# jyf588/SimGAN

Hardware: AMD Instinct MI355X
Metric: env-steps/sec of GAIL-dyn PPO update (higher is better)
Workload: dtype f32; 1 GPU; northstar: GAIL-dyn update, T=128 N=512/GPU obs=47 act=12 D-in=86 policy=mlp h64 D h100 ppo_epoch=10 num_mini_batch=1...; optimizer_steps_per_update=2720, parallelism=single GPU

## Files before the change

simgan_amd/csrc/sg_ppo.hip:

```cpp
#include <math.h>
#include <stdlib.h>
#include <string.h>

#include <algorithm>
#include <vector>

#include "sg_common.h"
#include "sg_rng.hpp"
#include "sg_ppo_kernels.hpp"
#include "sg_kfac.hpp"
#include "sg_gru_kernels.hpp"

__global__ void k_fill_perm(int64_t* perm, int64_t n, int half_bits, uint64_t key) {
    const int64_t i = (int64_t)blockIdx.x * blockDim.x + threadIdx.x;
    if (i < n) perm[i] = sg_perm_at(i, n, half_bits, key);
}

int sg_fill_perm(sg_ctx* ctx, int64_t* d_perm, int64_t n, uint64_t seed, uint64_t stream_id) {
    const uint64_t key = sg_key(seed, 0x5045524Dull, stream_id);
    hipLaunchKernelGGL(k_fill_perm, dim3((unsigned)((n + 255) / 256)), dim3(256), 0, ctx->stream, d_perm, n,
                       sg_perm_half_bits((uint64_t)n), key);
    SG_CHECK(hipGetLastError());
    return 0;
}

static int max_trunk_floats(const SgPolicyDesc& d) {
    int m = 0;
    for (int t = 0; t < d.n_trunks; ++t) m = d.trunk[t].size > m ? d.trunk[t].size : m;
    return m;
}
static int max_bwd_floats(const SgPolicyDesc& d) {
    int m = 0;
    for (int t = 0; t < d.n_trunks; ++t) { const int s = d.trunk[t].size - d.trunk[t].w2; m = s > m ? s : m; }
    return m;
}
static int stack_ldP(const SgPolicyDesc& d) {
    int m = 0;
    for (int t = 0; t < d.n_trunks; ++t) m = d.trunk[t].ldP > m ? d.trunk[t].ldP : m;
    return m;
}
static size_t ppo_fwd_lds(const SgPolicyDesc& d, int MT, bool gw) {
    const int R = 16 * MT;
    return sizeof(float) * ((gw ? 0 : (size_t)max_trunk_floats(d)) + R * d.ldO + 2 * R * d.ldH);
}
static bool ppo_fused(const SgPolicyDesc& d, int MT) {
    const char* e = getenv("SG_PPO_FUSED");
    return d.kind == SG_POLICY_MLP && MT <= 2 && !(e && !strcmp(e, "0"));
}
static size_t ppo_bwd_lds(const SgPolicyDesc& d, int MT, bool gw) {
    const int R = 16 * MT;
    return sizeof(float) * ((gw ? 0 : (size_t)(ppo_fused(d, MT) ? max_trunk_floats(d) : max_bwd_floats(d))) + R * d.ldO + 2 * R * d.ldH + 2 * R * stack_ldP(d) +
                            ((R * d.A + 3) & ~3) + 7 * R);
}
static size_t ppo_bwd_sym_lds(const SgPolicyDesc& d, int MT, bool gw) {
    const int R = 16 * MT;
    return sizeof(float) * ((gw ? 0 : (size_t)max_bwd_floats(d)) + R * d.ldO + 2 * R * d.ldH + 3 * R * stack_ldP(d) +
                            ((R * d.A + 3) & ~3) + 7 * R + ((d.A * d.A + 3) & ~3));
}

static size_t a2c_bwd_lds(const SgPolicyDesc& d, int MT, bool gw) {
    const int R = 16 * MT;
    return sizeof(float) * ((gw ? 0 : (size_t)max_bwd_floats(d)) + R * d.ldO + 2 * R * d.ldH + 2 * R * stack_ldP(d) +
                            ((R * d.A + 3) & ~3) + 7 * R);
}
#define SG_A2C_CHUNK_ROWS 4096

#define SG_PPO_SHAPES(X) X(1, 3, 4) X(2, 3, 4)  X(2, 1, 7)  \
                         X(2, 4, 7)  X(2, 7, 4)

static int ppo_block_threads(int MT) {
    const char* we = getenv("SG_PPO_WAVES");
    return (MT >= 2 && !(we && atoi(we) == 4)) ? 512 : 256;
}

static void launch_ppo_fwd(sg_ctx* ctx, int MT, const SgPolicyDesc& d, dim3 grid, size_t lds, const PpoArgs& pa, bool gw) {
    const int ko = d.Op / 16, kh = d.Hc == d.H ? d.Hp / 16 : 0;
// ... 1059 lines not shown
            for (int k = 0; k < M; ++k) {
                step_off[(size_t)e * M + k] = (int)n_own;
                for (int64_t i = 0; i < mb_global; ++i) {
                    const int64_t g = perms[(size_t)e * TN_perm + (size_t)k * mb_global + i];
                    const int64_t t = g / Ng, c = g - t * Ng, owner = c / r->N;
                    if (owner == ctx->rank) {
                        SG_REQUIRE(n_own < TN, "sg_ppo_update: epoch %d hands this rank more than its %lld rows", e, (long long)TN);
                        own_perm[(size_t)e * TN + n_own++] = t * r->N + (c - owner * r->N);
                    }
                }
                const int cnt = (int)n_own - step_off[(size_t)e * M + k];
                step_cnt[(size_t)e * M + k] = cnt;
                if (cnt > mb) mb = cnt;
            }
            epoch_rows[e] = n_own;
        }
    } else {
        for (int e = 0; e < E; ++e)
            for (int k = 0; k < M; ++k) { step_cnt[(size_t)e * M + k] = mb; step_off[(size_t)e * M + k] = k * mb; }
    }

    const bool sym = a->sym_coef > 0.f;
    if (sym) {
        if (a->d_mobs_mat) {
            if (a->mrows_cap < TN * d.O) {
                SG_CHECK(hipStreamSynchronize(ctx->stream));
                if (a->d_mrows) SG_CHECK(sg_dev_free(a->d_mrows));
                SG_CHECK(sg_dev_malloc((void**)&a->d_mrows, sizeof(float) * TN * d.O));
                a->mrows_cap = TN * d.O;
            }
            hipLaunchKernelGGL(k_mirror_rows, dim3((unsigned)((TN * d.O + 255) / 256)), dim3(256), 0, ctx->stream,
                               r->d_field[SG_F_OBS], a->d_mobs_mat, a->d_mrows, TN, d.O);
            SG_CHECK(hipGetLastError());
        } else {
            SG_REQUIRE(a->mrows_host == TN * d.O, "sg_ppo_update: the symmetry loss takes its mirrored observations from the host: "
                       "sg_ppo_set_mirrored_obs must hand over %lld floats (T*N rows of %d) before every update (pending: %lld)",
                       (long long)(TN * d.O), d.O, (long long)a->mrows_host);
            a->mrows_host = 0;
        }
    }

    float* adv = r->d_field[SG_F_ADVANTAGES];
    double* stats = a->d_loss_acc + 4;
    hipLaunchKernelGGL(k_adv_stats, dim3(1), dim3(1024), 0, ctx->stream, r->d_field[SG_F_RETURNS],
                       r->d_field[SG_F_VALUE_PREDS], TN, adv, stats, 0);
    if (ctx->use_comm) SG_TRY(sg_comm_allreduce_f64(ctx, stats, 3));
    hipLaunchKernelGGL(k_adv_stats, dim3(1), dim3(1024), 0, ctx->stream, r->d_field[SG_F_RETURNS],
                       r->d_field[SG_F_VALUE_PREDS], TN, adv, stats, 1);
    if (ctx->use_comm) SG_TRY(sg_comm_allreduce_f64(ctx, stats + 1, 1));
    hipLaunchKernelGGL(k_adv_stats, dim3(64), dim3(1024), 0, ctx->stream, r->d_field[SG_F_RETURNS],
                       r->d_field[SG_F_VALUE_PREDS], TN, adv, stats, 2);
    SG_CHECK(hipGetLastError());

    if (a->perms_cap < (int64_t)E * TN) {
        SG_CHECK(hipStreamSynchronize(ctx->stream));
        if (a->d_perms) SG_CHECK(sg_dev_free(a->d_perms));
        SG_CHECK(sg_dev_malloc((void**)&a->d_perms, sizeof(int64_t) * (size_t)E * TN));
        a->perms_cap = (int64_t)E * TN;
    }
    a->last_perm_count = owned ? 0 : (int64_t)E * TN;
    if (owned) {
        SG_CHECK(hipMemcpyAsync(a->d_perms, own_perm.data(), sizeof(int64_t) * (size_t)E * TN, hipMemcpyHostToDevice, ctx->stream));
        SG_CHECK(hipStreamSynchronize(ctx->stream));
    } else if (perms) {
        SG_CHECK(hipMemcpyAsync(a->d_perms, perms, sizeof(int64_t) * (size_t)E * TN, hipMemcpyHostToDevice, ctx->stream));
        if (!out3) SG_CHECK(hipStreamSynchronize(ctx->stream));
    } else {
        for (int e = 0; e < E; ++e)
            SG_TRY(sg_fill_perm(ctx, a->d_perms + (size_t)e * TN, TN, seed, (uint64_t)e * 2654435761ull + (uint64_t)ctx->rank));
    }

    const int ncols = d.n_trunks + (sym ? 1 : 0);
    int MT = ((size_t)((mb + 15) / 16) * (size_t)(d.total + 8) * sizeof(float) > ((size_t)24 << 20) ||
              ((mb + 31) / 32) * ncols >= ctx->num_cu) ? 2 : 1;
    if (const char* e = getenv("SG_PPO_ROWS")) {
        const int v = atoi(e);
        if (v == 16 || v == 32 || v == 64) MT = v / 16;
    }
    const bool gw = sg_policy_needs_gw(ctx, d) || ppo_fwd_lds(d, 1, false) > (size_t)ctx->lds_bytes ||
                    ppo_bwd_lds(d, 1, false) > (size_t)ctx->lds_bytes || (sym && ppo_bwd_sym_lds(d, 1, false) > (size_t)ctx->lds_bytes);
    if ((gw || sym) && MT > 2) MT = 2;
    while (MT > 1 && (ppo_fwd_lds(d, MT, gw) > (size_t)ctx->lds_bytes || ppo_bwd_lds(d, MT, gw) > (size_t)ctx->lds_bytes ||
                      (sym && ppo_bwd_sym_lds(d, MT, gw) > (size_t)ctx->lds_bytes))) MT /= 2;
    const int R = 16 * MT;
    const int G = (mb + R - 1) / R;
    const int mbp = G * R;
    const int ldP = stack_ldP(d);
    const int slab_stride = (d.total + 8 + 63) & ~63;
    const int TNp = (int)TN + 64 + (owned ? mbp : 0);

    const size_t slab_f = (size_t)(sym ? 2 : 1) * G * slab_stride;
    const size_t xm_off = ((size_t)TNp * (d.ldO + d.A + 4) + 3) & ~(size_t)3;
    const size_t epoch_f = sym ? xm_off + (size_t)TNp * d.ldO : (size_t)TNp * (d.ldO + d.A + 4);
    const size_t stack_f = (size_t)ncols * mbp * (2 * (size_t)d.ldH + ldP);
    if (a->slabs_cap < slab_f || a->stacks_cap < epoch_f + stack_f) {
        SG_CHECK(hipStreamSynchronize(ctx->stream));
        if (a->d_slabs) SG_CHECK(sg_dev_free(a->d_slabs));
        if (a->d_stacks) SG_CHECK(sg_dev_free(a->d_stacks));
        SG_CHECK(sg_dev_malloc((void**)&a->d_slabs, sizeof(float) * slab_f));
        SG_CHECK(sg_dev_malloc((void**)&a->d_stacks, sizeof(float) * (epoch_f + stack_f)));
        a->slabs_cap = slab_f;
        a->stacks_cap = epoch_f + stack_f;
        a->scratch_key = 0;
    }
    const uint64_t key = ((uint64_t)G << 40) ^ ((uint64_t)slab_stride << 20) ^ ((uint64_t)mbp << 8) ^ (uint64_t)TNp ^ ((uint64_t)MT << 60) ^
                         ((uint64_t)sym << 63);
    if (a->scratch_key != key) {
        SG_CHECK(hipMemsetAsync(a->d_slabs, 0, sizeof(float) * slab_f, ctx->stream));
        SG_CHECK(hipMemsetAsync(a->d_stacks, 0, sizeof(float) * (epoch_f + stack_f), ctx->stream));
        a->scratch_key = key;
    }
    hipLaunchKernelGGL(k_zero_f64, dim3(1), dim3(64), 0, ctx->stream, a->d_loss_acc, 4);

    float* epX = a->d_stacks;
    float* epACT = epX + (size_t)TNp * d.ldO;
    float* epSC = epACT + (size_t)TNp * d.A;
    float* epXm = sym ? a->d_stacks + xm_off : nullptr;
    float* stk = a->d_stacks + epoch_f;

    EpochGatherArgs ga;
    ga.obs = r->d_field[SG_F_OBS]; ga.actions = r->d_field[SG_F_ACTIONS]; ga.old_logp = r->d_field[SG_F_LOGP];
    ga.adv = adv; ga.vpred = r->d_field[SG_F_VALUE_PREDS]; ga.ret = r->d_field[SG_F_RETURNS];
    ga.TN = TN; ga.O = d.O; ga.Op = d.Op; ga.ldO = d.ldO; ga.A = d.A; ga.sc_stride = TNp;
    ga.X = epX; ga.ACT = epACT; ga.SC = epSC;
    ga.mobs = sym ? a->d_mrows : nullptr; ga.Xm = epXm;

    PpoArgs pa;
    pa.d = d; pa.params = a->policy->d_params;
    pa.sc_stride = TNp; pa.mb = mb; pa.mbp = mbp; pa.inv_B = 1.0f / (float)mb_global;
    pa.clip = a->cfg.clip_param; pa.vcoef = a->cfg.value_loss_coef; pa.ecoef = a->cfg.entropy_coef;
    pa.use_clipped = a->cfg.use_clipped_value_loss;
    pa.slabs = a->d_slabs; pa.slab_stride = slab_stride; pa.ldP = ldP; pa.dbg = a->d_dbg;
    pa.st = reinterpret_cast<SgOptState*>(a->d_state); pa.G = G; pa.k1 = 0;
    pa.pair = a->d_pair;
    pa.Xm = nullptr; pa.MA = a->d_mact;
    pa.sym_c = sym ? (float)(2.0 * a->sym_coef / ((double)mb_global * d.A)) : 0.f;
    for (int t = 0; t < 3; ++t) {
        const bool on = t < ncols;
        pa.H1[t] = on ? stk : nullptr; if (on) stk += (size_t)mbp * d.ldH;
        pa.H2[t] = on ? stk : nullptr; if (on) stk += (size_t)mbp * d.ldH;
        pa.OUT[t] = on ? stk : nullptr; if (on) stk += (size_t)mbp * ldP;
    }
    const int wb_f = gw ? 0 : max_trunk_floats(d), wb_b = gw ? 0 : max_bwd_floats(d);
    const bool fused = !sym && ppo_fused(d, MT);
    const size_t lds_fc = sizeof(float) * ((size_t)wb_f + R * d.ldO + 2 * R * d.ldH + 2 * R * ldP + ((R * d.A + 3) & ~3) + 7 * R);
    const char* cfenv = getenv("SG_PPO_CRITIC_FIRST");
    const bool crit_first = !gw && !fused && d.kind == SG_POLICY_SPLIT && MT <= 2 && lds_fc <= (size_t)ctx->lds_bytes &&
                            (cfenv ? cfenv[0] == '1' : G * d.n_trunks > ctx->num_cu);
    const char* penv = getenv("SG_PPO_PAIR");
    const bool pair = !gw && !fused && !crit_first && d.kind == SG_POLICY_SPLIT && d.n_trunks == 3 && MT <= 2 &&
                      lds_fc <= (size_t)ctx->lds_bytes && 3 * G <= ctx->num_cu && 2 * ldP + 2 <= std::min(d.trunk[0].ldH, d.trunk[1].ldH) && !a->d_dbg &&
                      !a->self_wait_failed && (penv ? strcmp(penv, "0") != 0 : sg_ctx_exclusive(ctx));
    if (pair && !a->pair_primed) SG_CHECK(hipMemsetAsync(a->d_stacks, 0, sizeof(float) * (epoch_f + stack_f), ctx->stream));
    a->pair_primed = pair;
    const size_t lds_f = ppo_fwd_lds(d, MT, gw), lds_b = sym ? ppo_bwd_sym_lds(d, MT, gw) : ppo_bwd_lds(d, MT, gw);
    const int nblk = (d.total + 8 + 255) / 256;
    const int nblk_r = (d.total + 8 + SG_PPO_REDUCE_PARAMS - 1) / SG_PPO_REDUCE_PARAMS;
    SgOptState* st = reinterpret_cast<SgOptState*>(a->d_state);

    auto enqueue_steps = [&]() -> int {
        hipLaunchKernelGGL(k_opt_prepare_first, dim3(1), dim3(1), 0, ctx->stream, st);
        for (int e = 0; e < E; ++e) {
            ga.perm = a->d_perms + (size_t)e * TN;
            ga.TN = epoch_rows[e];
            if (ga.TN) hipLaunchKernelGGL(sym ? k_ppo_epoch_gather_sym : k_ppo_epoch_gather, dim3((unsigned)((ga.TN + 63) / 64)), dim3(256), 0,
                                          ctx->stream, ga);
            for (int k = 0; k < M; ++k) {
                const size_t rb = (size_t)step_off[(size_t)e * M + k];
                pa.mb = step_cnt[(size_t)e * M + k];
                pa.X = epX + rb * d.ldO; pa.ACT = epACT + rb * d.A; pa.SC = epSC + rb;
                if (sym) pa.Xm = epXm + rb * d.ldO;
                pa.k1 = e * M + k + 1;
                if (sym) {
                    pa.wbuf_floats = wb_f;
                    launch_ppo_fwd_sym(ctx, MT, d, dim3(G, 3), lds_f, pa, gw);
                    pa.wbuf_floats = wb_b;
                    launch_ppo_bwd_sym(ctx, MT, d, dim3(G, 3), lds_b, pa, gw);
                } else if (pair) {
                    pa.wbuf_floats = wb_f;
                    launch_ppo_pair(ctx, MT, d, G, lds_fc, pa);
                } else if (crit_first) {
                    pa.wbuf_floats = wb_f;
                    launch_ppo_fwd_critic(ctx, MT, d, dim3(G, d.n_trunks), lds_fc > lds_f ? lds_fc : lds_f, pa);
                    pa.wbuf_floats = wb_b;
                    launch_ppo_bwd(ctx, MT, d, dim3(G, d.n_trunks - 1), lds_b, pa, false, false);
                } else {
                    if (!fused) {
                        pa.wbuf_floats = wb_f;
                        launch_ppo_fwd(ctx, MT, d, dim3(G, d.n_trunks), lds_f, pa, gw);
                    }
                    pa.wbuf_floats = fused ? wb_f : wb_b;
                    launch_ppo_bwd(ctx, MT, d, dim3(G, d.n_trunks), lds_b, pa, fused, gw);
                }
                if (sym) SG_LAUNCH(ctx, SG_PROF_PPO_REDUCE, k_ppo_reduce_sym, dim3(nblk_r), dim3(256), 0, a->d_slabs, G, slab_stride,
                                   d.total, a->d_grad, a->d_part, d.trunk[0].off, d.trunk[0].off + d.trunk[0].ex);
                else SG_LAUNCH(ctx, SG_PROF_PPO_REDUCE, k_ppo_reduce, dim3(nblk_r), dim3(256), 0, a->d_slabs, G, slab_stride,
                               d.total, a->d_grad, a->d_part);
                if (ctx->use_comm) {
                    SG_TRY(sg_comm_allreduce_f32(ctx, a->d_grad, d.total + 8));
                    hipLaunchKernelGGL(k_sumsq, dim3(nblk), dim3(256), 0, ctx->stream, a->d_grad, d.total, a->d_part);
                }
                SG_LAUNCH(ctx, SG_PROF_PPO_ADAM, sym ? k_ppo_adam_sym : k_ppo_adam, dim3(nblk), dim3(256), 0, a->policy->d_params, a->d_m,
                          a->d_v, a->d_grad, a->d_part, ctx->use_comm ? nblk : nblk_r, d.total, st, e * M + k + 1, a->cfg.eps,
                          a->cfg.max_grad_norm, pa.inv_B, a->d_loss_acc);
            }
        }
        hipLaunchKernelGGL(k_opt_commit, dim3(1), dim3(1), 0, ctx->stream, st, E * M);
        return 0;
    };
    const char* genv = getenv("SG_PPO_GRAPH");
    const char* gcenv = getenv("SG_PPO_GRAPH_COMM");
    const bool comm_ok = !a->graph_refused && (!ctx->use_comm || (sg_comm_graph_ok(ctx) && !(gcenv && !strcmp(gcenv, "0"))));
    bool use_graph = comm_ok && !owned && !ctx->profile && !a->d_dbg && !(genv && !strcmp(genv, "0"));
    if (use_graph) {
        uint32_t fbits[6];
        const float fv[6] = {a->cfg.clip_param, a->cfg.value_loss_coef, a->cfg.entropy_coef, a->cfg.eps, a->cfg.max_grad_norm, pa.inv_B};
        memcpy(fbits, fv, sizeof fbits);
        uint32_t cbits;
        memcpy(&cbits, &a->sym_coef, sizeof cbits);
        const uint64_t key[18] = {(uint64_t)(uintptr_t)a->d_slabs, (uint64_t)(uintptr_t)a->d_stacks, (uint64_t)(uintptr_t)a->d_perms,
                                  (uint64_t)(uintptr_t)r->d_field[SG_F_OBS], (uint64_t)(uintptr_t)r->d_field[SG_F_ACTIONS],
                                  (uint64_t)(uintptr_t)r->d_field[SG_F_RETURNS], (uint64_t)(uintptr_t)a->policy->d_params,
                                  (uint64_t)TN, ((uint64_t)E << 32) | (uint64_t)M, ((uint64_t)MT << 32) | (uint64_t)G,
                                  ((uint64_t)fbits[0] << 32) | fbits[1], ((uint64_t)fbits[2] << 32) | fbits[3],
                                  ((uint64_t)fbits[4] << 32) | fbits[5], (uint64_t)a->cfg.use_clipped_value_loss,
                                  (uint64_t)(uintptr_t)r->d_field[SG_F_LOGP], 0x50504full + (fused ? 1 : 0) + (ctx->use_comm ? 2 : 0) + (crit_first ? 4 : 0) + (gw ? 8 : 0) + (pair ? 16 : 0) + (sg_comm_peer_on(ctx) ? 32 : 0) + (sym ? 64 : 0) + ((uint64_t)sg_comm_peer_generation(ctx) << 32),
                                  sym ? (uint64_t)(uintptr_t)a->d_mrows : 0, sym ? (uint64_t)cbits : 0};
        if (!a->steps_graph || memcmp(key, a->steps_graph_key, sizeof key) != 0) {
            if (a->steps_graph) { SG_CHECK(hipGraphExecDestroy(a->steps_graph)); a->steps_graph = nullptr; }
            if (sg_try_capture(ctx, &a->steps_graph, enqueue_steps) != 0) {
                a->graph_refused = true;
                use_graph = false;
            } else {
                memcpy(a->steps_graph_key, key, sizeof key);
            }
        }
        if (use_graph) SG_CHECK(hipGraphLaunch(a->steps_graph, ctx->stream));
    }
    if (!use_graph) SG_TRY(enqueue_steps());
    SG_CHECK(hipGetLastError());
    a->opt_t += (int64_t)E * M;
    if (!out3) return 0;
    double acc[3];
    SG_TRY(sg_ctx_fetch_f64(ctx, a->d_loss_acc, acc, 3));
    if (pair && (acc[0] != acc[0] || acc[1] != acc[1] || acc[2] != acc[2])) {
        unsigned err = 0;
        SG_COPY_SYNC(ctx, &err, a->d_pair + SG_PAIR_ERR_WORD, sizeof err, hipMemcpyDeviceToHost);
        if (err) {
            SG_CHECK(hipMemsetAsync(a->d_pair + SG_PAIR_ERR_WORD, 0, sizeof err, ctx->stream));
            a->self_wait_failed = true;
            SG_REQUIRE(false, "sg_ppo_update: a workgroup of k_ppo_pair waited %d s for its partner's words and gave "
                       "up (the policy's state is undefined; SG_PPO_PAIR=0 runs the multi-launch step)", (int)(SG_PAIR_TIMEOUT_TICKS / 100000000ll));
        }
    }
    const double nu = (double)E * M;
    for (int i = 0; i < 3; ++i) out3[i] = (float)(acc[i] / nu);
    return 0;
}

__global__ void k_publish(double* dst, const double* d_acc, const double* d_scal, const double* p_acc, double n_d, double n_p,
                          const unsigned* d_err, const unsigned* a_err, const unsigned* peer_err) {
    const int t = threadIdx.x;
    if (t < 3) dst[t] = d_acc ? d_acc[t] : 0.0;
    else if (t < 8) dst[t] = d_scal ? d_scal[t - 3] : 0.0;
    else if (t < 11) dst[t] = p_acc ? p_acc[t - 8] : 0.0;
    else if (t == 11) dst[t] = n_d;
    else if (t == 12) dst[t] = n_p;
    else if (t == 13) dst[t] = d_err ? (double)*d_err : 0.0;
    else if (t == 14) dst[t] = a_err ? (double)*a_err : 0.0;
    else if (t == 15) dst[t] = peer_err ? (double)__hip_atomic_load(peer_err, __ATOMIC_RELAXED, __HIP_MEMORY_SCOPE_AGENT) : 0.0;
}

extern "C" int sg_results_publish(sg_ctx* ctx, sg_disc* d, sg_ppo* a, int slot) {
    SG_REQUIRE(ctx && slot >= 0 && slot < SG_RESULT_SLOTS, "sg_results_publish: bad argument");
    SG_REQUIRE((!d || d->ctx == ctx) && (!a || a->ctx == ctx), "sg_results_publish: objects of another context");
    SG_CHECK(hipSetDevice(ctx->device));
    hipLaunchKernelGGL(k_publish, dim3(1), dim3(64), 0, ctx->stream, ctx->results + 16 * slot, d ? d->d_loss_acc : nullptr,
                       d ? d->d_scal : nullptr, a ? a->d_loss_acc : nullptr, d ? (double)d->last_n_d : 1.0,
                       a ? (double)a->cfg.ppo_epoch * a->cfg.num_mini_batch : 1.0,
// ... 47 lines not shown
```

simgan_amd/csrc/sg_ppo_kernels.hpp:

```cpp
#pragma once
#include "sg_common.h"
#include "sg_thin.hpp"

#define HALF_LOG_2PI 0.91893853320467274178f

struct PpoArgs {
    SgPolicyDesc d;
    const float* params;
    const float* X;
    const float* ACT;
    const float* SC;
    int sc_stride;
    int mb, mbp;
    float inv_B;
    float clip, vcoef, ecoef;
    int use_clipped;
    float* H1[3];
    float* H2[3];
    float* OUT[3];
    float* slabs;
    int slab_stride;
    int ldP;
    int wbuf_floats;
    long long* dbg;
    SgOptState* st;
    int k1, G;
    unsigned* pair;
    const float* Xm;
    const float* MA;
    float sym_c;
    float* DX[2] = {nullptr, nullptr};
};

#define SG_PAIR_BYTES 64
#define SG_PAIR_TIMEOUT_TICKS 300000000ll



#define SG_LDS_SYNC() asm volatile("s_waitcnt lgkmcnt(0)\n\ts_barrier" ::: "memory")

#define SG_PPO_STAMP(n) do { if (a.dbg && threadIdx.x == 0 && blockIdx.y == 0) a.dbg[blockIdx.x * 16 + (n)] = clock64(); } while (0)
#define SG_PPO_WALL(n) do { if (a.dbg && threadIdx.x == 0 && blockIdx.y < 2) a.dbg[(blockIdx.x + 512 * blockIdx.y) * 16 + (n)] = wall_clock64(); } while (0)

struct EpochGatherArgs {
    const float *obs, *actions, *old_logp, *adv, *vpred, *ret;
    const int64_t* perm;
    int64_t TN;
    int O, Op, ldO, A, sc_stride;
    float *X, *ACT, *SC;
    const float* mobs;
    float* Xm;
};

template <bool SYM = false, bool ROLLOUT_ORDER = false>
__device__ __forceinline__ void sg_ppo_epoch_gather_body(const EpochGatherArgs& a) {
    __shared__ int IDX[64];
    const int tid = threadIdx.x;
    const int64_t row0 = (int64_t)blockIdx.x * 64;
    if (tid < 64) {
        const int64_t rr = row0 + tid;
        const int idx = rr < a.TN ? (ROLLOUT_ORDER ? (int)rr : (int)a.perm[rr]) : -1;
        IDX[tid] = idx;
        if (ROLLOUT_ORDER) {
            if (idx >= 0) a.SC[3 * (size_t)a.sc_stride + rr] = a.ret[idx];
        } else if (idx >= 0) {
            a.SC[0 * (size_t)a.sc_stride + rr] = a.old_logp[idx];
            a.SC[1 * (size_t)a.sc_stride + rr] = a.adv[idx];
            a.SC[2 * (size_t)a.sc_stride + rr] = a.vpred[idx];
            a.SC[3 * (size_t)a.sc_stride + rr] = a.ret[idx];
        }
    }
    __syncthreads();
    for (int base = tid; base < 64 * a.Op; base += 8 * blockDim.x) {
        float v[8];
#pragma unroll
        for (int u = 0; u < 8; ++u) {
            const int i = base + u * blockDim.x;
            const int r = i / a.Op, c = i - r * a.Op;
            v[u] = (i < 64 * a.Op && IDX[r] >= 0 && c < a.O) ? a.obs[(size_t)IDX[r] * a.O + c] : 0.f;
        }
#pragma unroll
        for (int u = 0; u < 8; ++u) {
            const int i = base + u * blockDim.x;
            if (i < 64 * a.Op && IDX[i / a.Op] >= 0) a.X[(size_t)(row0 + i / a.Op) * a.ldO + (i % a.Op)] = v[u];
        }
        if (SYM) {
#pragma unroll
            for (int u = 0; u < 8; ++u) {
                const int i = base + u * blockDim.x;
                const int r = i / a.Op, c = i - r * a.Op;
                v[u] = (i < 64 * a.Op && IDX[r] >= 0 && c < a.O) ? a.mobs[(size_t)IDX[r] * a.O + c] : 0.f;
            }
#pragma unroll
            for (int u = 0; u < 8; ++u) {
                const int i = base + u * blockDim.x;
                if (i < 64 * a.Op && IDX[i / a.Op] >= 0) a.Xm[(size_t)(row0 + i / a.Op) * a.ldO + (i % a.Op)] = v[u];
            }
        }
    }
    for (int i = tid; i < 64 * a.A; i += blockDim.x) {
        const int r = i / a.A, c = i - r * a.A;
        if (IDX[r] >= 0) a.ACT[(size_t)(row0 + r) * a.A + c] = a.actions[(size_t)IDX[r] * a.A + c];
    }
}

__global__ __launch_bounds__(256) void k_ppo_epoch_gather(EpochGatherArgs a) { sg_ppo_epoch_gather_body<false>(a); }
__global__ __launch_bounds__(256) void k_ppo_epoch_gather_sym(EpochGatherArgs a) { sg_ppo_epoch_gather_body<true>(a); }
__global__ __launch_bounds__(256) void k_a2c_gather(EpochGatherArgs a) { sg_ppo_epoch_gather_body<false, true>(a); }

__global__ __launch_bounds__(256) void k_mirror_rows(const float* obs, const float* m, float* out, int64_t rows, int O) {
    const int64_t idx = (int64_t)blockIdx.x * blockDim.x + threadIdx.x;
    if (idx >= rows * O) return;
    const int64_t r = idx / O;
    const int i = (int)(idx - r * O);
    const float* x = obs + r * O;
    const float* mi = m + (size_t)i * O;
    double s = 0.0;
    for (int j = 0; j < O; ++j) {
        const float w = mi[j];
        if (w != 0.f) s += (double)w * (double)x[j];
    }
    out[idx] = (float)s;
}

template <int MT, int KO, int KH, bool GW = false, bool SYM = false>
__device__ __forceinline__ void sg_ppo_fwd_body(const PpoArgs& a, const int t, const int bx) {
    extern __shared__ __attribute__((aligned(16))) float smem[];
    constexpr int R = 16 * MT;
    const SgPolicyDesc& d = a.d;
    const int tid = threadIdx.x;
    const bool mirror = SYM && t == 2;
    const SgTrunk tr = d.trunk[mirror ? 0 : t];
    const int Op = (KO > 0 && KH > 0) ? 16 * KO : d.Op, Hp = (KO > 0 && KH > 0) ? 16 * KH : tr.Hp;
    const int ldO = Op + 4, ldH = Hp + 4, ldP = a.ldP;
    const float* W = GW ? a.params + tr.off : smem;
    float* X = smem + a.wbuf_floats;
    float* H1 = X + R * ldO;
    float* H2 = H1 + R * ldH;
    const int row0 = bx * R;

    SG_PPO_STAMP(0);
    float4 wv[12];
    if (!GW) sg_stage_issue<12>(wv, a.params + tr.off, tr.size / 4);
    {
        const float4* gx = reinterpret_cast<const float4*>((mirror ? a.Xm : a.X) + (size_t)row0 * ldO);
        float4* lx = reinterpret_cast<float4*>(X);
        for (int i = tid; i < R * ldO / 4; i += blockDim.x) lx[i] = gx[i];
    }
    SG_PPO_STAMP(1);
    if (!GW) sg_stage_commit<12>(smem, wv, a.params + tr.off, tr.size / 4);
    __syncthreads();
    SG_PPO_STAMP(2);
    const float* b1 = W + tr.b1;
    const float* b2 = W + tr.b2;
    const float* bh = W + tr.bh;
    float* gH1 = a.H1[t] + (size_t)row0 * ldH;
    float* gH2 = a.H2[t] + (size_t)row0 * ldH;
    float* gOUT = a.OUT[t] + (size_t)row0 * ldP;
    sg_layer_nt_u<MT, GW>(X, ldO, W + tr.w1, ldO, Op, Hp, [&](int r, int c, float v) {
        const float h = sg_tanh(v + b1[c]);
        H1[r * ldH + c] = h;
// ... 407 lines not shown

template <int MT, int KO, int KH>
__global__ __launch_bounds__(512) void k_ppo_fwd_critic(PpoArgs a) {
    if (blockIdx.y == 0) sg_ppo_bwd_body<MT, KO, KH, true>(a, a.d.n_trunks - 1, blockIdx.x);
    else sg_ppo_fwd_body<MT, KO, KH>(a, blockIdx.y - 1, blockIdx.x);
}

#define SG_PPO_REDUCE_PARAMS 64
template <bool SYM, bool ACC = false>
__device__ __forceinline__ void sg_ppo_reduce_body(const float* slabs, int n_slabs_, int slab_stride, int total,
                                                   float* grad, float* part, int lo2, int hi2, int acc = 0) {
    __shared__ float red[4][64];
    const int lane = threadIdx.x & 63, wave = threadIdx.x >> 6;
    const int i = blockIdx.x * SG_PPO_REDUCE_PARAMS + lane;
    const int n_slabs = (SYM && i >= lo2 && i < hi2) ? 2 * n_slabs_ : n_slabs_;
    float g = 0.f;
    if (i < total + 8) {
        for (int s0 = wave; s0 < n_slabs; s0 += 64) {
            float t[16];
#pragma unroll
            for (int u = 0; u < 16; ++u) {
                const int sidx = s0 + 4 * u;
                t[u] = slabs[(size_t)(sidx < n_slabs ? sidx : s0) * slab_stride + i];
            }
#pragma unroll
            for (int u = 0; u < 16; ++u) g += (s0 + 4 * u < n_slabs) ? t[u] : 0.f;
        }
    }
    red[wave][lane] = g;
    __syncthreads();
    if (wave == 0) {
        g = (red[0][lane] + red[1][lane]) + (red[2][lane] + red[3][lane]);
        if (ACC && acc && i < total + 8) g += grad[i];
        if (i < total + 8) grad[i] = g;
        float sq = (i < total) ? g * g : 0.f;
        sq = sg_wave_sum(sq);
        if (lane == 0) part[blockIdx.x] = sq;
    }
}
__global__ __launch_bounds__(256) void k_ppo_reduce(const float* slabs, int n_slabs, int slab_stride, int total,
                                                    float* grad, float* part) {
    sg_ppo_reduce_body<false>(slabs, n_slabs, slab_stride, total, grad, part, 0, 0);
}
__global__ __launch_bounds__(256) void k_ppo_reduce_sym(const float* slabs, int n_slabs, int slab_stride, int total,
                                                        float* grad, float* part, int lo2, int hi2) {
    sg_ppo_reduce_body<true>(slabs, n_slabs, slab_stride, total, grad, part, lo2, hi2);
}
__global__ __launch_bounds__(256) void k_a2c_reduce(const float* slabs, int n_slabs, int slab_stride, int total,
                                                    float* grad, float* part, int acc) {
    sg_ppo_reduce_body<false, true>(slabs, n_slabs, slab_stride, total, grad, part, 0, 0, acc);
}

__global__ void k_opt_prepare_first(SgOptState* st) { sg_opt_prepare(st, st->t0 + 1); }

__global__ __launch_bounds__(256) void k_sumsq(const float* grad, int total, float* part) {
    const int i = blockIdx.x * blockDim.x + threadIdx.x;
    float sq = (i < total) ? grad[i] * grad[i] : 0.f;
    sq = sg_wave_sum(sq);
    __shared__ float ws[4];
    if ((threadIdx.x & 63) == 0) ws[threadIdx.x >> 6] = sq;
    __syncthreads();
    if (threadIdx.x == 0) part[blockIdx.x] = ws[0] + ws[1] + ws[2] + ws[3];
}

template <int NL>
__device__ __forceinline__ void sg_ppo_adam_body(float* params, float* m, float* v, const float* grad,
                                                 const float* part, int n_part, int total,
                                                 const SgOptState* st, int k1, float eps, float max_norm,
                                                 float inv_mb, double* loss_acc) {
    __shared__ float s_coef;
    const int t = st->t0 + k1;
    const float s_step_size = st->step_size2[t & 1], s_bc2_sqrt = st->bc2_sqrt2[t & 1];
    __shared__ float s_ws[4];
    {
        float s = 0.f;
        for (int j = threadIdx.x; j < n_part; j += 256) s += part[j];
        s = sg_wave_sum(s);
        if ((threadIdx.x & 63) == 0) s_ws[threadIdx.x >> 6] = s;
    }
    __syncthreads();
    if (threadIdx.x == 0) {
        const float norm = sqrtf((s_ws[0] + s_ws[1]) + (s_ws[2] + s_ws[3]));
        float coef = max_norm / (norm + 1e-6f);
        s_coef = coef > 1.f ? 1.f : coef;
    }
    __syncthreads();
    const int i = blockIdx.x * blockDim.x + threadIdx.x;
    if (i < total) {
        const float g = grad[i] * s_coef;
        float mi = m[i], vi = v[i];
        mi = mi + (g - mi) * (float)(1.0 - 0.9);
        vi = vi * (float)0.999 + (float)(1.0 - 0.999) * g * g;
        const float denom = sqrtf(vi) / s_bc2_sqrt + eps;
        params[i] = params[i] - s_step_size * (mi / denom);
        m[i] = mi;
        v[i] = vi;
    }
    if (blockIdx.x == 0 && threadIdx.x < NL)
        loss_acc[threadIdx.x] += (double)(grad[total + threadIdx.x] * inv_mb);
    if (blockIdx.x == 0 && threadIdx.x == 64) sg_opt_prepare(const_cast<SgOptState*>(st), t + 1);
}
__global__ __launch_bounds__(256) void k_ppo_adam(float* params, float* m, float* v, const float* grad,
                                                  const float* part, int n_part, int total,
                                                  const SgOptState* st, int k1, float eps, float max_norm,
                                                  float inv_mb, double* loss_acc) {
    sg_ppo_adam_body<3>(params, m, v, grad, part, n_part, total, st, k1, eps, max_norm, inv_mb, loss_acc);
}
__global__ __launch_bounds__(256) void k_ppo_adam_sym(float* params, float* m, float* v, const float* grad,
                                                      const float* part, int n_part, int total,
                                                      const SgOptState* st, int k1, float eps, float max_norm,
                                                      float inv_mb, double* loss_acc) {
    sg_ppo_adam_body<4>(params, m, v, grad, part, n_part, total, st, k1, eps, max_norm, inv_mb, loss_acc);
}

__global__ __launch_bounds__(256) void k_a2c_rmsprop(float* params, float* sq, const float* grad, const float* part, int n_part,
                                                     int total, const SgOptState* st, float alpha, float one_m_alpha, float eps,
                                                     float max_norm, float inv_b, double* loss_acc) {
    __shared__ float s_coef;
    __shared__ float s_ws[4];
    {
        float s = 0.f;
        for (int j = threadIdx.x; j < n_part; j += 256) s += part[j];
        s = sg_wave_sum(s);
        if ((threadIdx.x & 63) == 0) s_ws[threadIdx.x >> 6] = s;
    }
    __syncthreads();
    if (threadIdx.x == 0) {
        const float norm = sqrtf((s_ws[0] + s_ws[1]) + (s_ws[2] + s_ws[3]));
        const float coef = max_norm / (norm + 1e-6f);
        s_coef = coef > 1.f ? 1.f : coef;
    }
    __syncthreads();
    const int i = blockIdx.x * blockDim.x + threadIdx.x;
    if (i < total) {
        const float g = grad[i] * s_coef;
        const float s = sq[i] * alpha + one_m_alpha * g * g;
        params[i] = params[i] + (-st->lr) * (g / (sqrtf(s) + eps));
        sq[i] = s;
    }
    if (blockIdx.x == 0 && threadIdx.x < 3) loss_acc[threadIdx.x] += (double)(grad[total + threadIdx.x] * inv_b);
}

__global__ __launch_bounds__(1024) void k_adv_stats(const float* ret, const float* vpred, int64_t n, float* adv,
                                                    double* stats ,
                                                    int pass) {
    __shared__ double ws[16];
    __shared__ double s_mean;
    const int tid = threadIdx.x;
    if (pass == 0) {
        double s = 0.0;
        for (int64_t i = tid; i < n; i += blockDim.x) {
            const float a = ret[i] - vpred[i];
            adv[i] = a;
            s += (double)a;
        }
        s = sg_wave_sum(s);
        if ((tid & 63) == 0) ws[tid >> 6] = s;
        __syncthreads();
        if (tid == 0) {
            double t = 0.0;
// ... 29 lines not shown
```

Baseline: 2.519 million env-steps/s.

## Overlap next-epoch gather with Adam steps via double-buffered epoch scratch

Double-buffers the per-epoch gathered minibatch scratch and spreads the next epoch's gather blocks across the Adam kernel launches of the current epoch, so the separate gather launch at each epoch boundary disappears. It also fills all epoch permutations in one 2-D launch, merges loss-accumulator zeroing into the optimizer prologue kernel, and restructures the gather body so scalar and action loads are issued before the observation copy. The change costs extra scratch memory and adds blocks to the Adam launches, and it is gated by an environment variable that defaults on.

Result: no change. 2.524 million env-steps/s, median of 4 (+0.2%).

```diff
diff --git a/simgan_amd/csrc/sg_ppo.hip b/simgan_amd/csrc/sg_ppo.hip
--- a/simgan_amd/csrc/sg_ppo.hip
+++ b/simgan_amd/csrc/sg_ppo.hip
@@ -22,6 +22,26 @@
                        sg_perm_half_bits((uint64_t)n), key);
     SG_CHECK(hipGetLastError());
     return 0;
+}
+
+__global__ void k_fill_perms(int64_t* perm, int64_t n, int half_bits, uint64_t seed, uint64_t stream0, uint64_t stride) {
+    const int64_t i = (int64_t)blockIdx.x * blockDim.x + threadIdx.x;
+    const uint64_t key = sg_key(seed, 0x5045524Dull, stream0 + (uint64_t)blockIdx.y * stride);
+    if (i < n) perm[(int64_t)blockIdx.y * n + i] = sg_perm_at(i, n, half_bits, key);
+}
+
+static int sg_fill_perms(sg_ctx* ctx, int64_t* d_perm, int64_t n, int E, uint64_t seed, uint64_t stream0, uint64_t stride) {
+    hipLaunchKernelGGL(k_fill_perms, dim3((unsigned)((n + 255) / 256), (unsigned)E), dim3(256), 0, ctx->stream, d_perm, n,
+                       sg_perm_half_bits((uint64_t)n), seed, stream0, stride);
+    SG_CHECK(hipGetLastError());
+    return 0;
+}
+
+static int ppo_epoch_pipeline() {
+    const char* e = getenv("SG_PPO_EPOCH_PIPELINE");
+    if (!e) return 16;
+    const int v = atoi(e);
+    return v == 0 ? 0 : v == 64 ? 64 : 16;
 }
 
 static int max_trunk_floats(const SgPolicyDesc& d) {
@@ -1187,6 +1207,7 @@
                        r->d_field[SG_F_VALUE_PREDS], TN, adv, stats, 2);
     SG_CHECK(hipGetLastError());
 
+    const int pipe_rows = ppo_epoch_pipeline();
     if (a->perms_cap < (int64_t)E * TN) {
         SG_CHECK(hipStreamSynchronize(ctx->stream));
         if (a->d_perms) SG_CHECK(sg_dev_free(a->d_perms));
@@ -1200,6 +1221,8 @@
     } else if (perms) {
         SG_CHECK(hipMemcpyAsync(a->d_perms, perms, sizeof(int64_t) * (size_t)E * TN, hipMemcpyHostToDevice, ctx->stream));
         if (!out3) SG_CHECK(hipStreamSynchronize(ctx->stream));
+    } else if (pipe_rows) {
+        SG_TRY(sg_fill_perms(ctx, a->d_perms, TN, E, seed, (uint64_t)ctx->rank, 2654435761ull));
     } else {
         for (int e = 0; e < E; ++e)
             SG_TRY(sg_fill_perm(ctx, a->d_perms + (size_t)e * TN, TN, seed, (uint64_t)e * 2654435761ull + (uint64_t)ctx->rank));
@@ -1228,30 +1251,34 @@
     const size_t xm_off = ((size_t)TNp * (d.ldO + d.A + 4) + 3) & ~(size_t)3;
     const size_t epoch_f = sym ? xm_off + (size_t)TNp * d.ldO : (size_t)TNp * (d.ldO + d.A + 4);
     const size_t stack_f = (size_t)ncols * mbp * (2 * (size_t)d.ldH + ldP);
-    if (a->slabs_cap < slab_f || a->stacks_cap < epoch_f + stack_f) {
+    const bool pipe = pipe_rows && !sym && !owned && E > 1;
+    const size_t ep2_off = (epoch_f + stack_f + 63) & ~(size_t)63;
+    const size_t scratch_f = pipe ? ep2_off + epoch_f : epoch_f + stack_f;
+    if (a->slabs_cap < slab_f || a->stacks_cap < scratch_f) {
         SG_CHECK(hipStreamSynchronize(ctx->stream));
         if (a->d_slabs) SG_CHECK(sg_dev_free(a->d_slabs));
         if (a->d_stacks) SG_CHECK(sg_dev_free(a->d_stacks));
         SG_CHECK(sg_dev_malloc((void**)&a->d_slabs, sizeof(float) * slab_f));
-        SG_CHECK(sg_dev_malloc((void**)&a->d_stacks, sizeof(float) * (epoch_f + stack_f)));
+        SG_CHECK(sg_dev_malloc((void**)&a->d_stacks, sizeof(float) * scratch_f));
         a->slabs_cap = slab_f;
-        a->stacks_cap = epoch_f + stack_f;
+        a->stacks_cap = scratch_f;
         a->scratch_key = 0;
     }
     const uint64_t key = ((uint64_t)G << 40) ^ ((uint64_t)slab_stride << 20) ^ ((uint64_t)mbp << 8) ^ (uint64_t)TNp ^ ((uint64_t)MT << 60) ^
-                         ((uint64_t)sym << 63);
+                         ((uint64_t)sym << 63) ^ ((uint64_t)pipe << 59);
     if (a->scratch_key != key) {
         SG_CHECK(hipMemsetAsync(a->d_slabs, 0, sizeof(float) * slab_f, ctx->stream));
-        SG_CHECK(hipMemsetAsync(a->d_stacks, 0, sizeof(float) * (epoch_f + stack_f), ctx->stream));
+        SG_CHECK(hipMemsetAsync(a->d_stacks, 0, sizeof(float) * scratch_f, ctx->stream));
         a->scratch_key = key;
     }
-    hipLaunchKernelGGL(k_zero_f64, dim3(1), dim3(64), 0, ctx->stream, a->d_loss_acc, 4);
+    if (!pipe_rows) hipLaunchKernelGGL(k_zero_f64, dim3(1), dim3(64), 0, ctx->stream, a->d_loss_acc, 4);
 
     float* epX = a->d_stacks;
     float* epACT = epX + (size_t)TNp * d.ldO;
     float* epSC = epACT + (size_t)TNp * d.A;
     float* epXm = sym ? a->d_stacks + xm_off : nullptr;
     float* stk = a->d_stacks + epoch_f;
+    const size_t ep_flip = pipe ? ep2_off : 0;
 
     EpochGatherArgs ga;
     ga.obs = r->d_field[SG_F_OBS]; ga.actions = r->d_field[SG_F_ACTIONS]; ga.old_logp = r->d_field[SG_F_LOGP];
@@ -1294,16 +1321,29 @@
     SgOptState* st = reinterpret_cast<SgOptState*>(a->d_state);
 
     auto enqueue_steps = [&]() -> int {
-        hipLaunchKernelGGL(k_opt_prepare_first, dim3(1), dim3(1), 0, ctx->stream, st);
+        if (pipe_rows) hipLaunchKernelGGL(k_ppo_prologue, dim3(1), dim3(64), 0, ctx->stream, st, a->d_loss_acc, 4);
+        else hipLaunchKernelGGL(k_opt_prepare_first, dim3(1), dim3(1), 0, ctx->stream, st);
         for (int e = 0; e < E; ++e) {
+            const size_t cur = (e & 1) ? ep_flip : 0, nxt = ep_flip - cur;
             ga.perm = a->d_perms + (size_t)e * TN;
             ga.TN = epoch_rows[e];
-            if (ga.TN) hipLaunchKernelGGL(sym ? k_ppo_epoch_gather_sym : k_ppo_epoch_gather, dim3((unsigned)((ga.TN + 63) / 64)), dim3(256), 0,
-                                          ctx->stream, ga);
+            ga.X = epX + cur; ga.ACT = epACT + cur; ga.SC = epSC + cur;
+            if (ga.TN && (e == 0 || !pipe))
+                hipLaunchKernelGGL(sym ? k_ppo_epoch_gather_sym : k_ppo_epoch_gather, dim3((unsigned)((ga.TN + 63) / 64)), dim3(256), 0,
+                                   ctx->stream, ga);
+            EpochGatherArgs gn = ga;
+            int ride_blocks = 0, ride_per = 0;
+            if (pipe && e + 1 < E) {
+                gn.perm = a->d_perms + (size_t)(e + 1) * TN;
+                gn.TN = epoch_rows[e + 1];
+                gn.X = epX + nxt; gn.ACT = epACT + nxt; gn.SC = epSC + nxt;
+                ride_blocks = (int)((gn.TN + pipe_rows - 1) / pipe_rows);
+                ride_per = (ride_blocks + M - 1) / M;
+            }
             for (int k = 0; k < M; ++k) {
                 const size_t rb = (size_t)step_off[(size_t)e * M + k];
                 pa.mb = step_cnt[(size_t)e * M + k];
-                pa.X = epX + rb * d.ldO; pa.ACT = epACT + rb * d.A; pa.SC = epSC + rb;
+                pa.X = epX + cur + rb * d.ldO; pa.ACT = epACT + cur + rb * d.A; pa.SC = epSC + cur + rb;
                 if (sym) pa.Xm = epXm + rb * d.ldO;
                 pa.k1 = e * M + k + 1;
                 if (sym) {
@@ -1335,9 +1375,19 @@
                     SG_TRY(sg_comm_allreduce_f32(ctx, a->d_grad, d.total + 8));
                     hipLaunchKernelGGL(k_sumsq, dim3(nblk), dim3(256), 0, ctx->stream, a->d_grad, d.total, a->d_part);
                 }
-                SG_LAUNCH(ctx, SG_PROF_PPO_ADAM, sym ? k_ppo_adam_sym : k_ppo_adam, dim3(nblk), dim3(256), 0, a->policy->d_params, a->d_m,
-                          a->d_v, a->d_grad, a->d_part, ctx->use_comm ? nblk : nblk_r, d.total, st, e * M + k + 1, a->cfg.eps,
-                          a->cfg.max_grad_norm, pa.inv_B, a->d_loss_acc);
+                const int g0 = k * ride_per, g_blocks = std::max(0, std::min(ride_per, ride_blocks - g0));
+                if (g_blocks > 0 && pipe_rows == 64)
+                    SG_LAUNCH(ctx, SG_PROF_PPO_ADAM, k_ppo_adam_gather<64>, dim3(nblk + g_blocks), dim3(256), 0, a->policy->d_params, a->d_m,
+                              a->d_v, a->d_grad, a->d_part, ctx->use_comm ? nblk : nblk_r, d.total, st, e * M + k + 1, a->cfg.eps,
+                              a->cfg.max_grad_norm, pa.inv_B, a->d_loss_acc, gn, nblk, g0);
+                else if (g_blocks > 0)
+                    SG_LAUNCH(ctx, SG_PROF_PPO_ADAM, k_ppo_adam_gather<16>, dim3(nblk + g_blocks), dim3(256), 0, a->policy->d_params, a->d_m,
+                              a->d_v, a->d_grad, a->d_part, ctx->use_comm ? nblk : nblk_r, d.total, st, e * M + k + 1, a->cfg.eps,
+                              a->cfg.max_grad_norm, pa.inv_B, a->d_loss_acc, gn, nblk, g0);
+                else
+                    SG_LAUNCH(ctx, SG_PROF_PPO_ADAM, sym ? k_ppo_adam_sym : k_ppo_adam, dim3(nblk), dim3(256), 0, a->policy->d_params, a->d_m,
+                              a->d_v, a->d_grad, a->d_part, ctx->use_comm ? nblk : nblk_r, d.total, st, e * M + k + 1, a->cfg.eps,
+                              a->cfg.max_grad_norm, pa.inv_B, a->d_loss_acc);
             }
         }
         hipLaunchKernelGGL(k_opt_commit, dim3(1), dim3(1), 0, ctx->stream, st, E * M);
@@ -1359,7 +1409,7 @@
                                   (uint64_t)TN, ((uint64_t)E << 32) | (uint64_t)M, ((uint64_t)MT << 32) | (uint64_t)G,
                                   ((uint64_t)fbits[0] << 32) | fbits[1], ((uint64_t)fbits[2] << 32) | fbits[3],
                                   ((uint64_t)fbits[4] << 32) | fbits[5], (uint64_t)a->cfg.use_clipped_value_loss,
-                                  (uint64_t)(uintptr_t)r->d_field[SG_F_LOGP], 0x50504full + (fused ? 1 : 0) + (ctx->use_comm ? 2 : 0) + (crit_first ? 4 : 0) + (gw ? 8 : 0) + (pair ? 16 : 0) + (sg_comm_peer_on(ctx) ? 32 : 0) + (sym ? 64 : 0) + ((uint64_t)sg_comm_peer_generation(ctx) << 32),
+                                  (uint64_t)(uintptr_t)r->d_field[SG_F_LOGP], 0x50504full + (fused ? 1 : 0) + (ctx->use_comm ? 2 : 0) + (crit_first ? 4 : 0) + (gw ? 8 : 0) + (pair ? 16 : 0) + (sg_comm_peer_on(ctx) ? 32 : 0) + (sym ? 64 : 0) + ((uint64_t)pipe_rows << 8) + ((uint64_t)sg_comm_peer_generation(ctx) << 32),
                                   sym ? (uint64_t)(uintptr_t)a->d_mrows : 0, sym ? (uint64_t)cbits : 0};
         if (!a->steps_graph || memcmp(key, a->steps_graph_key, sizeof key) != 0) {
             if (a->steps_graph) { SG_CHECK(hipGraphExecDestroy(a->steps_graph)); a->steps_graph = nullptr; }
diff --git a/simgan_amd/csrc/sg_ppo_kernels.hpp b/simgan_amd/csrc/sg_ppo_kernels.hpp
--- a/simgan_amd/csrc/sg_ppo_kernels.hpp
+++ b/simgan_amd/csrc/sg_ppo_kernels.hpp
@@ -52,61 +52,70 @@
     float* Xm;
 };
 
-template <bool SYM = false, bool ROLLOUT_ORDER = false>
-__device__ __forceinline__ void sg_ppo_epoch_gather_body(const EpochGatherArgs& a) {
-    __shared__ int IDX[64];
+template <bool SYM = false, bool ROLLOUT_ORDER = false, int ROWS = 64>
+__device__ __forceinline__ void sg_ppo_epoch_gather_body(const EpochGatherArgs& a, int blk) {
+    __shared__ int IDX[ROWS];
     const int tid = threadIdx.x;
-    const int64_t row0 = (int64_t)blockIdx.x * 64;
-    if (tid < 64) {
+    const int64_t row0 = (int64_t)blk * ROWS;
+    if (tid < ROWS) {
         const int64_t rr = row0 + tid;
-        const int idx = rr < a.TN ? (ROLLOUT_ORDER ? (int)rr : (int)a.perm[rr]) : -1;
-        IDX[tid] = idx;
-        if (ROLLOUT_ORDER) {
-            if (idx >= 0) a.SC[3 * (size_t)a.sc_stride + rr] = a.ret[idx];
-        } else if (idx >= 0) {
-            a.SC[0 * (size_t)a.sc_stride + rr] = a.old_logp[idx];
-            a.SC[1 * (size_t)a.sc_stride + rr] = a.adv[idx];
-            a.SC[2 * (size_t)a.sc_stride + rr] = a.vpred[idx];
-            a.SC[3 * (size_t)a.sc_stride + rr] = a.ret[idx];
-        }
-    }
-    __syncthreads();
-    for (int base = tid; base < 64 * a.Op; base += 8 * blockDim.x) {
+        IDX[tid] = rr < a.TN ? (ROLLOUT_ORDER ? (int)rr : (int)a.perm[rr]) : -1;
+    }
+    __syncthreads();
+    float sc[4] = {0.f, 0.f, 0.f, 0.f};
+    const int my_idx = tid < ROWS ? IDX[tid] : -1;
+    if (my_idx >= 0) {
+        if (!ROLLOUT_ORDER) { sc[0] = a.old_logp[my_idx]; sc[1] = a.adv[my_idx]; sc[2] = a.vpred[my_idx]; }
+        sc[3] = a.ret[my_idx];
+    }
+    const bool act0 = tid < ROWS * a.A && IDX[tid / a.A] >= 0;
+    const float av0 = act0 ? a.actions[(size_t)IDX[tid / a.A] * a.A + (tid % a.A)] : 0.f;
+    for (int base = tid; base < ROWS * a.Op; base += 8 * blockDim.x) {
         float v[8];
 #pragma unroll
         for (int u = 0; u < 8; ++u) {
             const int i = base + u * blockDim.x;
             const int r = i / a.Op, c = i - r * a.Op;
-            v[u] = (i < 64 * a.Op && IDX[r] >= 0 && c < a.O) ? a.obs[(size_t)IDX[r] * a.O + c] : 0.f;
+            v[u] = (i < ROWS * a.Op && IDX[r] >= 0 && c < a.O) ? a.obs[(size_t)IDX[r] * a.O + c] : 0.f;
         }
 #pragma unroll
         for (int u = 0; u < 8; ++u) {
             const int i = base + u * blockDim.x;
-            if (i < 64 * a.Op && IDX[i / a.Op] >= 0) a.X[(size_t)(row0 + i / a.Op) * a.ldO + (i % a.Op)] = v[u];
+            if (i < ROWS * a.Op && IDX[i / a.Op] >= 0) a.X[(size_t)(row0 + i / a.Op) * a.ldO + (i % a.Op)] = v[u];
         }
         if (SYM) {
 #pragma unroll
             for (int u = 0; u < 8; ++u) {
                 const int i = base + u * blockDim.x;
                 const int r = i / a.Op, c = i - r * a.Op;
-                v[u] = (i < 64 * a.Op && IDX[r] >= 0 && c < a.O) ? a.mobs[(size_t)IDX[r] * a.O + c] : 0.f;
+                v[u] = (i < ROWS * a.Op && IDX[r] >= 0 && c < a.O) ? a.mobs[(size_t)IDX[r] * a.O + c] : 0.f;
             }
 #pragma unroll
             for (int u = 0; u < 8; ++u) {
                 const int i = base + u * blockDim.x;
-                if (i < 64 * a.Op && IDX[i / a.Op] >= 0) a.Xm[(size_t)(row0 + i / a.Op) * a.ldO + (i % a.Op)] = v[u];
-            }
-        }
-    }
-    for (int i = tid; i < 64 * a.A; i += blockDim.x) {
+                if (i < ROWS * a.Op && IDX[i / a.Op] >= 0) a.Xm[(size_t)(row0 + i / a.Op) * a.ldO + (i % a.Op)] = v[u];
+            }
+        }
+    }
+    if (my_idx >= 0) {
+        const int64_t rr = row0 + tid;
+        if (!ROLLOUT_ORDER) {
+            a.SC[0 * (size_t)a.sc_stride + rr] = sc[0];
+            a.SC[1 * (size_t)a.sc_stride + rr] = sc[1];
+            a.SC[2 * (size_t)a.sc_stride + rr] = sc[2];
+        }
+        a.SC[3 * (size_t)a.sc_stride + rr] = sc[3];
+    }
+    if (act0) a.ACT[(size_t)(row0 + tid / a.A) * a.A + (tid % a.A)] = av0;
+    for (int i = tid + blockDim.x; i < ROWS * a.A; i += blockDim.x) {
         const int r = i / a.A, c = i - r * a.A;
         if (IDX[r] >= 0) a.ACT[(size_t)(row0 + r) * a.A + c] = a.actions[(size_t)IDX[r] * a.A + c];
     }
 }
 
-__global__ __launch_bounds__(256) void k_ppo_epoch_gather(EpochGatherArgs a) { sg_ppo_epoch_gather_body<false>(a); }
-__global__ __launch_bounds__(256) void k_ppo_epoch_gather_sym(EpochGatherArgs a) { sg_ppo_epoch_gather_body<true>(a); }
-__global__ __launch_bounds__(256) void k_a2c_gather(EpochGatherArgs a) { sg_ppo_epoch_gather_body<false, true>(a); }
+__global__ __launch_bounds__(256) void k_ppo_epoch_gather(EpochGatherArgs a) { sg_ppo_epoch_gather_body<false>(a, blockIdx.x); }
+__global__ __launch_bounds__(256) void k_ppo_epoch_gather_sym(EpochGatherArgs a) { sg_ppo_epoch_gather_body<true>(a, blockIdx.x); }
+__global__ __launch_bounds__(256) void k_a2c_gather(EpochGatherArgs a) { sg_ppo_epoch_gather_body<false, true>(a, blockIdx.x); }
 
 __global__ __launch_bounds__(256) void k_mirror_rows(const float* obs, const float* m, float* out, int64_t rows, int O) {
     const int64_t idx = (int64_t)blockIdx.x * blockDim.x + threadIdx.x;
@@ -620,6 +629,10 @@
 }
 
 __global__ void k_opt_prepare_first(SgOptState* st) { sg_opt_prepare(st, st->t0 + 1); }
+__global__ void k_ppo_prologue(SgOptState* st, double* loss_acc, int n_loss) {
+    if (threadIdx.x == 0) sg_opt_prepare(st, st->t0 + 1);
+    if ((int)threadIdx.x < n_loss) loss_acc[threadIdx.x] = 0.0;
+}
 
 __global__ __launch_bounds__(256) void k_sumsq(const float* grad, int total, float* part) {
     const int i = blockIdx.x * blockDim.x + threadIdx.x;
@@ -674,6 +687,17 @@
                                                   float inv_mb, double* loss_acc) {
     sg_ppo_adam_body<3>(params, m, v, grad, part, n_part, total, st, k1, eps, max_norm, inv_mb, loss_acc);
 }
+template <int ROWS>
+__global__ __launch_bounds__(256) void k_ppo_adam_gather(float* params, float* m, float* v, const float* grad,
+                                                         const float* part, int n_part, int total,
+                                                         const SgOptState* st, int k1, float eps, float max_norm,
+                                                         float inv_mb, double* loss_acc, EpochGatherArgs ga, int n_adam, int gblk0) {
+    if ((int)blockIdx.x >= n_adam) {
+        sg_ppo_epoch_gather_body<false, false, ROWS>(ga, gblk0 + ((int)blockIdx.x - n_adam));
+        return;
+    }
+    sg_ppo_adam_body<3>(params, m, v, grad, part, n_part, total, st, k1, eps, max_norm, inv_mb, loss_acc);
+}
 __global__ __launch_bounds__(256) void k_ppo_adam_sym(float* params, float* m, float* v, const float* grad,
                                                       const float* part, int n_part, int total,
                                                       const SgOptState* st, int k1, float eps, float max_norm,
```
